# spectrseq/spectrseqtools

Hardware: AMD Instinct MI355X
Metric: peaks explained/sec (full 148-nt alphabet, <=20-mer) at 1/2/4/8 MI355X (higher is better)
Workload: dtype u64; 1 GPU; config3: synthetic spectra (SURVEY 8(d)), full 104-mass/105-row alphabet, <=20-mer, A7 (4 breakages/peak) + A8 (sliding-window differences) per step; spectra_per_gpu=10000, max_len=20, max_modifications=10, a7_stream=engine stream, parallelism=1 GPU

## Files before the change

include/sst.h:

```cpp
#ifndef SST_H
#define SST_H

#include <stdint.h>

#ifdef __cplusplus
extern "C" {
#endif

#define SST_OK 0
#define SST_E_ARG (-1)
#define SST_E_HIP (-2)
#define SST_E_NOMEM (-3)
#define SST_E_TABLE (-4)
#define SST_E_INTERNAL (-5)

#define SST_NONE 0
#define SST_EMPTY 1
#define SST_SOME 2
#define SST_OUT_OF_TABLE (-1)
#define SST_OVERFLOW (-2)
#define SST_ABORTED (-4)


typedef struct sst_ctx sst_ctx;
// ... 68 lines not shown
int sst_step_rows_device(sst_table* t, const double* d_obs, const int64_t* d_peak_off, int64_t n_spec,
                         int64_t n_peaks, const double* d_intensity, double intensity_cutoff, double mass_cutoff,
                         const double* d_su_seq, const double* shifts, const uint8_t* sides, int n_shifts,
                         double max_weight, double tolerance, double precision, int64_t max_mods_scalar,
                         uint64_t cap_per_query, int64_t max_queries, int8_t* d_valid_out, sst_result** out);
int sst_result_queries(sst_result* r, int64_t* n);

int sst_result_settle(sst_result* r, uint64_t* n_hits, uint64_t* payload_bytes);

int sst_result_host(sst_result* r, const int8_t** status, const uint64_t** count, const uint64_t** offset,
                    const uint8_t** payload, uint64_t* payload_bytes);
int sst_result_device(sst_result* r, int8_t** d_status, uint64_t** d_count, uint64_t** d_offset,
                      uint8_t** d_payload, uint64_t* payload_bytes);
int sst_result_hit_list(sst_result* r, void** d_hits, uint64_t* n_hits);
int sst_result_pair_hits(sst_result* r, void** d_refs, uint64_t* n_pair_hits, uint64_t* pair_bytes, int* n_scan_wg);
int sst_table_pair_records(sst_table* t, uint32_t* recs, int64_t cap, int64_t* n);
int64_t sst_wire_pack(sst_result* r, const int8_t* d_valid, int64_t n_valid, void* d_out, int64_t cap);
int sst_result_fetch(sst_result* r);
void sst_result_free(sst_result* r);

int sst_result_stats(const sst_result* r, uint64_t* stats_out );

#define SST_LB_EMPTY_WINDOW (-5)
int sst_length_bound_alpha_batch(sst_table* t, const double* su_mass, const double* obs_mass, const int32_t* spec,
                                 const uint64_t* alpha, int64_t n_alpha, int64_t n, double tolerance,
                                 double precision, int max_len, int64_t max_mods, int direction, int64_t* out,
                                 int8_t* status);
#define SST_LB_EXACT_ONLY 2
#define SST_LB_REPLAY 4
int sst_length_bound_batch(sst_table* t, const double* su_mass, const double* obs_mass, int64_t n, double tolerance,
// ... 314 lines not shown
```

spectrseqtools_amd/_native.py:

```python
import ctypes
import os
import threading

import numpy as np

_HERE = os.path.dirname(os.path.abspath(__file__))
LIB_PATH = os.environ.get("SST_LIBRARY", os.path.join(_HERE, "libsstgpu.so"))

SST_NONE, SST_EMPTY, SST_SOME = 0, 1, 2
SST_OUT_OF_TABLE, SST_OVERFLOW, SST_ABORTED = -1, -2, -4
SST_LB_EMPTY_WINDOW = -5

EXPORTS = (
    "sst_device_count", "sst_ctx_create", "sst_ctx_destroy", "sst_last_error", "sst_ctx_stream",
    "sst_ctx_synchronize", "sst_table_build", "sst_table_upload", "sst_table_set_budgets", "sst_table_shape",
    "sst_table_download", "sst_table_destroy", "sst_is_valid_batch", "sst_is_valid_batch_device",
    "sst_explain_batch", "sst_explain_batch_device", "sst_explain_alpha_batch_device", "sst_explain_alpha_lens_batch_device", "sst_result_host", "sst_result_device", "sst_result_fetch",
    "sst_result_free", "sst_result_stats", "sst_profile_enable", "sst_profile_select",
    "sst_profile_sample", "sst_profile_read", "sst_length_bound_batch", "sst_explain_recursion_batch", "sst_is_singleton_batch",
    "sst_is_singleton_batch_device", "sst_ctx_set_stream", "sst_result_hit_list", "sst_result_settle",
    "sst_window_pairs", "sst_is_valid_peaks", "sst_is_valid_peaks_device", "sst_result_pair_hits",
    "sst_table_pair_records", "sst_su_diff_queries", "sst_sort_rows", "sst_step_device",
    "sst_wire_pack", "sst_explain_pairs_alpha", "sst_explain_pairs_alpha_device", "sst_is_valid_alpha",
    "sst_is_valid_alpha_device", "sst_dict_union", "sst_step_rows_device", "sst_result_queries",
    "sst_classify_rows_device", "sst_fix_round_device", "sst_valid_rows_alpha_device",
    "sst_bins_count_device", "sst_bins_emit_device", "sst_length_bound_alpha_batch",
    "sst_py_tuple_hash", "sst_pyset_order", "sst_pyset_table_size", "sst_walk_scratch_bytes",
    "sst_skel_walk_device", "sst_result_refs_device", "sst_dict_count_device", "sst_dict_build_device",
    "sst_reach_rows_device", "sst_length_bounds_reach_device", "sst_jaccard_device", "sst_skeleton_alpha_device",
    "sst_dict_list_device", "sst_fix_finish_device", "sst_pipe_reserve_rows", "sst_reach_lowest_device",
    "sst_length_bounds_frontier_device", "sst_post_skeleton_device", "sst_ctx_trim", "sst_requery_merge_device",
    "sst_handoff_count_device", "sst_handoff_emit_device",
)

K_IS_VALID, K_EXPLAIN_SCAN, K_EXPLAIN_DEEP, K_EXPLAIN_NOMEMO, K_EXPLAIN_EXACT, K_EXPLAIN_EXPAND = 0, 1, 2, 3, 4, 5
K_RESULT_PACK = 6
(K_CLASSIFY_ROWS, K_FIX_ROUND, K_VALID_ALPHA, K_BINS_COUNT, K_BINS_EMIT, K_DICT, K_SKEL_WALK, K_REACH_ROWS,
 K_LENGTH_BOUND, K_JACCARD, K_PAIRS_ALPHA, K_REQUERY_MERGE, K_HANDOFF) = range(7, 20)
K_COUNT = 24
KERNEL_NAMES = {K_IS_VALID: "k_is_valid", K_EXPLAIN_SCAN: "k_explain_scan", K_EXPLAIN_DEEP: "k_explain_deferred",
                K_EXPLAIN_EXPAND: "k_explain_expand",
                K_RESULT_PACK: "k_result_pack",
                K_CLASSIFY_ROWS: "k_classify_rows", K_FIX_ROUND: "k_fix_round", K_VALID_ALPHA: "k_valid_alpha",
                K_BINS_COUNT: "k_bins_count", K_BINS_EMIT: "k_bins_emit", K_DICT: "k_dict_build",
                K_SKEL_WALK: "k_skel_walk", K_REACH_ROWS: "k_reach_rows", K_LENGTH_BOUND: "k_length_bound",
                K_JACCARD: "k_jaccard", K_PAIRS_ALPHA: "k_pairs_alpha", K_REQUERY_MERGE: "k_requery_merge",
                K_HANDOFF: "k_handoff"}
# ... 156 lines not shown
    lib.sst_profile_enable.argtypes = [_P, _I]
    lib.sst_profile_select.argtypes = [_P, ctypes.c_uint32]
    lib.sst_profile_sample.argtypes = [_P, ctypes.c_uint32]
    lib.sst_profile_read.argtypes = [_P, _P, _P]
    lib.sst_length_bound_batch.argtypes = [_P, _P, _P, _I64, _D, _D, _I, _I64, _I, _P, _P]
    lib.sst_length_bound_alpha_batch.argtypes = [_P, _P, _P, _P, _P, _I64, _I64, _D, _D, _I, _I64, _I, _P, _P]
    lib.sst_explain_recursion_batch.argtypes = [_P, _P, _P, _I64, _D, _D, _P, _I64, _U64, _PP]
    lib.sst_is_singleton_batch.argtypes = [_P, _P, _I, _P, _P, _I64, _D, _D, _P]
    lib.sst_is_singleton_batch_device.argtypes = [_P, _P, _I, _P, _P, _I64, _D, _D, _P]
    lib.sst_is_valid_peaks.argtypes = [_P, _P, _I64, _P, _I, _D, _D, _P]
    lib.sst_is_valid_peaks_device.argtypes = [_P, _P, _I64, _P, _I, _D, _D, _P]
    lib.sst_window_pairs.argtypes = [_P, _P, _I64, _D, _P, _P, _I64]
    lib.sst_window_pairs.restype = _I64
    lib.sst_result_pair_hits.argtypes = [_P, _PP, ctypes.POINTER(_U64), ctypes.POINTER(_U64), ctypes.POINTER(_I)]
    lib.sst_result_pair_hits.restype = _I
    lib.sst_table_pair_records.argtypes = [_P, _P, _I64, ctypes.POINTER(_I64)]
    lib.sst_table_pair_records.restype = _I
    lib.sst_wire_pack.argtypes = [_P, _P, _I64, _P, _I64]
    lib.sst_wire_pack.restype = _I64
    lib.sst_su_diff_queries.argtypes = [_P, _P, _P, _P, _I64, _D, _D, _P, _P, _P, _P, _I64]
    lib.sst_su_diff_queries.restype = _I64
    lib.sst_py_tuple_hash.argtypes = [_P, _I64]
    lib.sst_py_tuple_hash.restype = _I64
    lib.sst_pyset_order.argtypes = [_P, _P, _I64, _P]
    lib.sst_pyset_order.restype = _I64
    lib.sst_sort_rows.argtypes = [_P, _P, _I64, _I64, _P]
    lib.sst_sort_rows.restype = _I
    lib.sst_step_device.argtypes = [_P, _P, _I64, _P, _I, _P, _P, _P, _I64, _D, _D, _P, _I64, _I, _U64, _PP]
    lib.sst_step_device.restype = _I
    lib.sst_explain_pairs_alpha.argtypes = [_P, _P, _P, _P, _P, _I64, _I64, _D, _D, _P, _P, _P, _P]
# ... 400 lines not shown
    def _wrap(cls, engine, h, w):
        nr, nc, C = _I(), _I64(), _I()
        engine._lib.sst_table_shape(h, ctypes.byref(nr), ctypes.byref(nc), ctypes.byref(C))
        return cls(engine, h, nr.value, nc.value, C.value, w.tolist())

    def set_budgets(self, is_mod, caps):
        key = (tuple(bool(x) for x in is_mod), tuple(int(c) for c in caps))
        if key == self._budgets:
            return
        m = np.ascontiguousarray(key[0], dtype=np.uint8)
        c = np.ascontiguousarray(key[1], dtype=np.int64)
        self.engine.check(self.engine._lib.sst_table_set_budgets(self.handle, _ptr(m), _ptr(c)),
                          "sst_table_set_budgets")
        self._budgets = key

    def pair_records(self):
        L = self.engine._lib
        n = _I64()
        self.engine.check(L.sst_table_pair_records(self.handle, None, 0, ctypes.byref(n)), "sst_table_pair_records")
        out = np.zeros(n.value, np.uint32)
        if n.value:
            self.engine.check(L.sst_table_pair_records(self.handle, _ptr(out), n.value, ctypes.byref(n)),
                              "sst_table_pair_records")
        return out

    def download(self):
        out = np.empty((self.n_rows, self.n_cols), dtype=_DT[self.compression])
        self.engine.check(self.engine._lib.sst_table_download(self.handle, _ptr(out)), "sst_table_download")
        return out

# ... 241 lines not shown
```

spectrseqtools_amd/csrc/sst_api.cpp:

```cpp
#include <hip/hip_runtime.h>
#include <sched.h>

#include <algorithm>
#include <atomic>
#include <chrono>
#include <cmath>
#include <cstdio>
#include <cstdlib>
#include <cstring>
#include <mutex>
#include <string>
#include <thread>
#include <vector>

#include "sst.h"
#include "sst_internal.h"
#include "sst_pyset.h"

using namespace sst;

namespace {

struct DevBuf {
  void* p = nullptr;
// ... 47 lines not shown
  DevBuf ws_deep;
  DevBuf ws_hash, ws_frames, ws_stacks, ws_epochs;
  DevBuf singleton_masses;
  struct LbfWs {
    DevBuf flags, lpar, lval, gtab, ctab, glist, ctl, bstart, bgroups, qi, qrow, roots, ncnt, grec, crec, ngrp;
    uint64_t S = 0, ncap = 0, budget = 0;
    bool by_default = false;
    int epoch = 0;
    bool dirty = true;
    uint64_t done_q = 0, done_nodes = 0;
    double band_frac = 0.3;
  } lbf, lbf_small;
  uint32_t hash_cap = 0;
  int exact_blocks = 0;
  int n_cu = 256;
  int expand_blocks = 0;
  uint32_t prof = 0;
  struct Pending {
    int kid;
    hipEvent_t a, b;
  };
  std::vector<Pending> pending;
  std::vector<hipEvent_t> pool;
  double prof_ms[SST_K_COUNT] = {0};
  int64_t prof_n[SST_K_COUNT] = {0};
  uint32_t prof_every = 1;
  uint64_t prof_seen[SST_K_COUNT] = {0};
  DevBuf pipe_big;
  uint32_t pipe_big_rows = 0, pipe_big_slots = 0;
  int pipe_big_wg = 0;
// ... 2 lines not shown
struct sst_table {
  sst_ctx* ctx = nullptr;
  int n_rows = 0;
  int64_t n_cols = 0;
  int C = 32;
  int64_t M = 0;
  std::vector<int64_t> masses;
  std::vector<uint8_t> is_mod;
  std::vector<int64_t> cap;
  DevBuf packed, index, valid, w, capd, modd, pairs, census, canon_c;
  int64_t canon_c_words = 0;
  std::vector<uint32_t> pair_recs;
  uint64_t pair_key = 0;
  bool pair_key_set = false;
  int scan_blocks = 0;
  bool closure = false;
  TableArgs args{};
};

struct LenBudgets {
  const int32_t* qlen = nullptr;
  const int32_t* caps = nullptr;
  const uint64_t* capz = nullptr;
  const uint32_t* never = nullptr;
};

struct sst_result {
  sst_ctx* ctx = nullptr;
  int64_t n = 0;
  int64_t cap_n = 0;
// ... 313 lines not shown
  *out = nullptr;
  int n = sst_device_count();
  if (device < 0 || device >= n) return SST_E_ARG;
  sst_ctx* c = new sst_ctx();
  c->device = device;
  {
    int cu = 0;
    if (hipDeviceGetAttribute(&cu, hipDeviceAttributeMultiprocessorCount, device) == hipSuccess && cu > 0) c->n_cu = cu;
    (void)hipGetLastError();
  }
  if (hipSetDevice(device) != hipSuccess || hipStreamCreateWithFlags(&c->own, hipStreamNonBlocking) != hipSuccess) {
    delete c;
    return SST_E_HIP;
  }
  c->stream = c->own;
  *out = c;
  return SST_OK;
}

void sst_ctx_destroy(sst_ctx* c) {
  if (!c) return;
  (void)hipSetDevice(c->device);
  (void)hipStreamSynchronize(c->stream);
  (void)hipStreamSynchronize(c->own);
  for (DevBuf* b : {&c->in_mass, &c->in_thr, &c->in_mods, &c->out_valid, &c->ws_deep, &c->ws_hash, &c->ws_frames,
                    &c->ws_stacks, &c->ws_epochs, &c->singleton_masses})
    b->release();
  prof_resolve(c);
  for (hipEvent_t e : c->pool) (void)hipEventDestroy(e);
  (void)hipStreamDestroy(c->own);
// ... 532 lines not shown
  fold_scan_limits(ta, q);
  q.alpha = d_alpha;
  q.spec = d_spec;
  q.comp = (int)t->C;
  q.qlen = lb.qlen;
  q.caps_len = lb.caps;
  q.capz_len = lb.capz;
  q.never_len = lb.never;
  OutArgs o = out_args(r);
  const bool fused = !eager_tail && !r->bitset_scan;
  r->fused_pass = fused;
  r->scan_hdr_pending = fused;
  r->scan_hits = r->scan_bytes = 0;
  if (fused) {
    o.fused = 1;
    o.pass_id = ++r->pack_seq;
#ifdef SST_DIAG
    static const char* dbg = getenv("SST_PACK_DBG");
    o.dbg = dbg ? atoi(dbg) : 0;
#endif
  }
  const bool step = peaks && peaks->n > 0 && peaks->n_shifts == 4 && fused;
  if (peaks && peaks->n > 0 && peaks->n_shifts > 0 && !step) {
    Prof p(c, SST_K_IS_VALID);
    HIP_OK(c, launch_is_valid_peaks(t->args.valid, t->args.limit, t->args.full_lo, t->args.full_hi,
                                    t->args.first_reach, peaks->obs, peaks->n, peaks->shifts, peaks->n_shifts, tol,
                                    prec, peaks->out, c->stream));
  }
  {
    Prof p(c, SST_K_EXPLAIN_MAIN);
// ... 10 lines not shown
    eager_tail = true;
  }
  if (eager_tail)
    if (int rc = launch_tail(t, r)) return rc;
  return launch_pack(r);
}

int step_scan_wg_per_cu() {
  static const int v = [] {
    const char* e = getenv("SST_STEP_SCAN_WG_PER_CU");
    return e && atoi(e) > 0 ? atoi(e) : 1;
  }();
  return v;
}

int alloc_result(sst_table* t, int64_t n, sst_result** out, bool step = false) {
  sst_ctx* c = t->ctx;
  if (t->scan_blocks == 0) t->scan_blocks = c->n_cu * explain_scan_blocks_per_cu(scan_dyn_lds(t->args));
  if (c->expand_blocks == 0) c->expand_blocks = c->n_cu * explain_expand_blocks_per_cu();
  sst_result* r = new sst_result();
  r->ctx = c;
  r->pass_stream = c->stream;
  r->n = n;
  r->cap_n = n;
  size_t nn = (size_t)std::max<int64_t>(n, 1);
  int64_t tiles = ((int64_t)nn + 63) / 64;
  const int64_t grid = step ? (int64_t)c->n_cu * std::min<int64_t>(t->scan_blocks / c->n_cu, step_scan_wg_per_cu())
                            : (int64_t)t->scan_blocks;
  r->n_wg = (int)std::max<int64_t>(1, std::min<int64_t>(grid, (tiles + 15) / 16));
  r->n_scan_waves = (int64_t)r->n_wg * (kScanWG / 64);
  r->work_region = (uint64_t)((tiles + r->n_scan_waves - 1) / r->n_scan_waves) * 64;
  r->n_expand_waves = c->expand_blocks * (kWG / 64);
  r->region_bytes = std::max<uint64_t>(2048, round16(16 * r->work_region));
// ... 611 lines not shown
  *n_hits = r->n_hits;
  return SST_OK;
}

int sst_result_pair_hits(sst_result* r, void** d_refs, uint64_t* n_pair_hits, uint64_t* pair_bytes, int* n_scan_wg) {
  if (!r) return SST_E_ARG;
  sst_ctx* c = r->ctx;
  std::lock_guard<std::recursive_mutex> g(c->mu);
  if (int rc = set_device(c)) return rc;
  if (int rc = settle(r)) return rc;
  if (int rc = order_after_settle(r)) return rc;
  if (d_refs) *d_refs = r->refs.p;
  if (n_pair_hits) *n_pair_hits = r->scan_hits;
  if (pair_bytes) *pair_bytes = r->scan_bytes;
  if (n_scan_wg) *n_scan_wg = r->rows_pass ? 0 : r->n_wg;
  return SST_OK;
}

int sst_table_pair_records(sst_table* t, uint32_t* recs, int64_t cap, int64_t* n) {
  if (!t || !n) return SST_E_ARG;
  *n = t->args.pairs_enabled ? (int64_t)t->pair_recs.size() : 0;
  if (!recs || *n == 0) return SST_OK;
  if (cap < *n) return fail(t->ctx, SST_E_ARG, "pair records: buffer too small");
  memcpy(recs, t->pair_recs.data(), (size_t)*n * 4);
  return SST_OK;
}

static uint64_t pair_key_of(const std::vector<uint32_t>& recs) {
  uint64_t h = 0xCBF29CE484222325ull;
  const uint8_t* p = (const uint8_t*)recs.data();
// ... 1727 lines not shown
```

spectrseqtools_amd/csrc/sst_internal.h:

```cpp
#pragma once
#include <hip/hip_runtime.h>
#include <stddef.h>
#include <stdint.h>

#include <type_traits>

#include "sst.h"

namespace sst {

constexpr int kMaxRows = 120;
static_assert(kMaxRows == SST_MAX_ROWS, "the ABI's row stride");
constexpr int kWG = 256;
#ifndef SST_DEF_WG
#define SST_DEF_WG 256
#endif
constexpr int kDefWG = SST_DEF_WG;
constexpr int kShallowDepth = 4;
constexpr int kMaxDepth = 96;
constexpr int kInfBudget = 1 << 30;
constexpr int kScanWG = 1024;
constexpr int kMaxSingletonMasses = 1024;
constexpr int kMaxPairLds = 44 * 1024;
constexpr uint32_t kItemZero = 1u, kItemUnclassified = 2u, kItemNever = 4u;
// ... 90 lines not shown
  uint32_t* counters;
  uint32_t* lists;
  unsigned long long* stats;
  uint4* dhits;
  uint32_t* dhit_count;
  int fused;
  uint64_t* agg;
  uint64_t* agg_next;
  uint4* hits_out;
  uint16_t* hit_refs;
  uint8_t* dense;
  uint64_t* hdr;
  uint64_t* hdr_host;
  uint64_t pass_id;
  int dbg;
};

constexpr uint32_t kHitOffsetFlag = 1u << 31;

enum {
  kCtlCursor = 0,
  kCtlCounters = 1,
  kCtlExactRetries = 3,
  kCtlArenaRetries = 13,
  kCtlRegionNeed = 14,
  kCtlStats = 256,
  kCtlDhits = 512,
  kCtlWords = 1024
};

enum {
// ... 425 lines not shown
                           const double* mass, const double* thr, int64_t n, double tol, double prec, int8_t* out,
                           hipStream_t st);
hipError_t launch_is_valid_peaks(const uint64_t* valid, int64_t limit, int64_t full_lo, int64_t full_hi,
                                 int64_t first_reach, const double* obs, int64_t n, const double* shifts, int n_w,
                                 double tol, double prec, int8_t* out, hipStream_t st);
hipError_t launch_step(const TableArgs& t, const QueryArgs& q, const OutArgs& o, int n_blocks, const double* obs,
                       int64_t n_peaks, const double* shifts4, double tol, double prec, int8_t* valid_out,
                       hipStream_t st);
hipError_t launch_explain_scan(const TableArgs& t, const QueryArgs& q, const OutArgs& o, int n_blocks,
                               hipStream_t st);
hipError_t launch_explain_expand(const TableArgs& t, const QueryArgs& q, const OutArgs& o, int n_blocks,
                                 hipStream_t st);
int explain_scan_blocks_per_cu(size_t dyn_lds);
int explain_expand_blocks_per_cu();
size_t scan_dyn_lds(const TableArgs& t);
hipError_t launch_result_pack(const PackArgs& p, hipStream_t st);
hipError_t launch_hits_to_arrays(const uint4* hits, uint64_t n_hits, const int8_t* status, uint64_t* count,
                                 uint64_t* offset, hipStream_t st);
hipError_t launch_explain_deferred(const TableArgs& t, const QueryArgs& q, const OutArgs& o, void* ws_deep,
                                   int shallow_blocks, int deep_blocks, const ExactWs& ws, int exact_blocks,
                                   hipStream_t st);
size_t glob_frame_bytes();
hipError_t launch_layer_step(const uint64_t* prev, uint64_t* next, int64_t nwords, const int* w, int n_rows,
                             hipStream_t st);
hipError_t launch_length_bound(const TableArgs& t, const LBArgs& q, char* hash, int8_t* vals, char* frames,
                               uint32_t hash_cap, int exact_units, bool fast_pass, hipStream_t st);
size_t lb_frame_bytes();
hipError_t launch_is_singleton(const int64_t* masses, int n_masses, const double* mass, const double* thr, int64_t n,
                               double tol, double prec, int8_t* out, hipStream_t st);
hipError_t launch_explain_recursion(const TableArgs& t, const QueryArgs& q, const OutArgs& o, char* hash,
// ... 8 lines not shown
```

spectrseqtools_amd/csrc/sst_kernels.hip:

```cpp
#include <hip/hip_runtime.h>
#include <stdint.h>

#include <algorithm>

#include "sst_internal.h"
#include "sst_quant.h"

namespace sst {

struct M128 {
  uint64_t a, b;
};
__device__ __forceinline__ M128 rows_upto(int r) {
  M128 m;
  if (r >= 63) {
    m.a = ~0ull;
    int k = r - 63;
    m.b = k >= 64 ? ~0ull : ((1ull << k) - 1ull);
  } else {
    m.a = r < 0 ? 0ull : ((2ull << r) - 1ull);
    m.b = 0;
  }
  return m;
}
// ... 1463 lines not shown
  asm volatile("" : "+s"(p));
  return p;
}
template <typename T>
__device__ __forceinline__ T karg_load(KargPtr p, size_t off) {
  static_assert(std::is_trivially_copyable<T>::value, "kernarg members are plain data");
  T v;
  __builtin_memcpy(&v, (const __attribute__((address_space(4))) T*)(p + off), sizeof(T));
  return v;
}
#define SCAN_KARG(p, member) \
  karg_load<std::remove_cv_t<decltype(((ScanArgs*)nullptr)->member)>>(p, offsetof(ScanArgs, member))

template <bool THR, bool MODS>
__device__ __forceinline__ void scan_end_phase(uint32_t bid, uint32_t nbid, uint32_t w_in, int lane, uint32_t n_hit,
                                               uint32_t n_staged, uint32_t n_work, uint32_t st_q,
                                               uint32_t st_payload);

template <bool THR, bool MODS>
__device__ __forceinline__ void explain_scan_wg(const ScanArgs& a, const uint32_t bid, const uint32_t nbid) {
  const TableArgs& t = a.t;
  const QueryArgs& q = a.q;
  const OutArgs& out = a.out;
  extern __shared__ uint32_t lds_pair_img[];
  if (bid == 0) {
    if (threadIdx.x < (unsigned)out.ctl_words) out.ctl_next[threadIdx.x] = 0;
    for (uint32_t k = threadIdx.x; k < nbid; k += blockDim.x) out.agg_next[k] = 0;
  }
  const int n_img = 2 * (t.n_pairs + 2) + t.n_buckets;
  static_assert(kMaxPairLds <= kImgPieces * kScanWG * 16, "the image is staged in kImgPieces pieces per lane");
  const uint32_t n_img16 = (uint32_t)(n_img + 3) >> 2;
  const __amdgpu_buffer_rsrc_t img_rsrc = buf_rsrc(t.pair_data, n_img16 * 16u);
  u32x4 img[kImgPieces];
#pragma unroll
  for (int j = 0; j < kImgPieces; ++j)
    img[j] = __builtin_amdgcn_raw_buffer_load_b128(img_rsrc, (threadIdx.x + j * kScanWG) * 16u, 0, 0);
  const PairLds pl = scan_pair_lds(lds_pair_img, t.n_pairs, t.pair_base, t.pair_shift);
  const int lane = threadIdx.x & 63;
  const uint32_t w_in = __builtin_amdgcn_readfirstlane(threadIdx.x >> 6);
  const uint32_t wave = bid * (kScanWG / 64) + w_in;
  const uint32_t n_waves = nbid * (kScanWG / 64);
  const uint32_t n = (uint32_t)q.n;
  const uint32_t ntiles = (n + 63) >> 6;
  const double limitf = (double)t.limit;
  uint32_t st_q = 0, st_payload = 0;
  uint4* wl = out.work + (uint64_t)wave * out.work_region;
  uint32_t n_work = 0;
  const uint32_t wl_bytes = (uint32_t)(out.work_region * 16);
  const __amdgpu_buffer_rsrc_t wl_rsrc = buf_rsrc(wl, wl_bytes);
  const __amdgpu_buffer_rsrc_t st_rsrc = buf_rsrc(out.status, n);
  uint32_t n_hit = 0;
  uint32_t n_staged = 0;
  auto fetch = [&](uint32_t tl, double& m, double& tt, int64_t& mm) {
    const uint32_t j = tl < ntiles ? min(tl * 64 + lane, n - 1) : n - 1;
    m = __builtin_nontemporal_load(q_at(q.mass, j));
    if (THR) tt = __builtin_nontemporal_load(q_at(q.thr, j));
    if (MODS) mm = __builtin_nontemporal_load(q_at(q.max_mods, j));
  };
  auto step = [&](uint32_t tile, double m_in, double t_in, int64_t mm_cur) {
    const uint32_t i = tile * 64 + lane;
    const bool live = i < n;
    const double m_cur = m_in, t_cur = THR ? t_in : q.tol * m_in;
    double lof, hif;
    quantise_lean_fn(m_cur, t_cur, [] { return SCAN_KARG(scan_karg(), q.prec); }, q.rprec, lof, hif);
    const bool nonempty = live && lof <= hif;
    const bool oot = nonempty && !(hif < limitf);
    const bool zero = nonempty && !oot && lof <= 0.0 && hif >= 0.0;
    const double af = __builtin_fmax(lof, 1.0);
    const bool active = nonempty && !oot && af <= hif;
    const uint32_t a = active ? (uint32_t)af : 0u, hi = active ? (uint32_t)hif : 0u;
    bool pair, a0ok = true;
    if (MODS) {
      const int A0 = clamp_budget(mm_cur);
      a0ok = !t.any_mod || A0 >= kInfBudget || (uint64_t)hi < (uint64_t)(A0 + 1) * (uint64_t)t.w_min_mod;
      pair = active && a0ok && hi < t.pair_lim;
    } else {
      pair = active && hi < q.pair_hi_lim;
    }
    const bool work = active && !pair;
    uint32_t first = 0, cnt = 0, bytes = 0;
    if (pair) cnt = pair_walk(pl, a, hi, first, bytes);
    int8_t status = oot ? (int8_t)SST_OUT_OF_TABLE : (zero ? (int8_t)SST_EMPTY : (int8_t)SST_NONE);
    if (cnt) status = cnt > q.cap32 ? (int8_t)SST_OVERFLOW : (int8_t)SST_SOME;
    st_payload += status == SST_SOME ? bytes + 2u : 0u;
    st_q += pair ? 1u : 0u;
    const uint64_t hbal = __ballot(cnt != 0);
    const uint32_t hpos = n_hit + mbcnt(hbal);
    __builtin_amdgcn_raw_buffer_store_b8((uint8_t)status, st_rsrc, (live && !work) ? i : kBufSkip, 0, 0);
    const u32x2 rv = {i, first | (cnt << 16)};
    __builtin_amdgcn_raw_buffer_store_b64(rv, wl_rsrc, cnt ? wl_bytes - 8u * (hpos + 1u) : kBufSkip, 0, 0);
    n_hit += (uint32_t)__builtin_popcountll(hbal);
    if (__ballot(work)) {
      const KargPtr ka = scan_karg();
      bool never;
      if (MODS) {
        const int32_t* const qlen = SCAN_KARG(ka, q.qlen);
        const uint32_t nl = qlen ? SCAN_KARG(ka, q.never_len)[qlen[live ? i : n - 1]] : SCAN_KARG(ka, t.never_lim);
        never = a0ok && hi < nl;
      } else {
        never = hi < SCAN_KARG(ka, q.never_hi_lim);
      }
      int cls = -1;
      if (work) {
        if (never && hi < SCAN_KARG(ka, t.shallow_hi)) {
          cls = kClassShallow;
        } else {
          cls = never ? kClassDeep : (SCAN_KARG(ka, q.with_memo) ? kClassExact : kClassNomemo);
          SCAN_KARG(ka, out.status)[i] = (int8_t)kStatusPending;
        }
      }
      uint32_t* const stage = SCAN_KARG(ka, out.stage) + (uint64_t)wave * SCAN_KARG(ka, out.work_region);
      const uint64_t cb = __ballot(cls >= 0);
      if (cls >= 0) stage[n_staged + mbcnt(cb)] = i | ((uint32_t)cls << 30);
      n_staged += (uint32_t)__builtin_popcountll(cb);
    }
  };
  double mA = 0.0, tA = 0.0, mB = 0.0, tB = 0.0;
  int64_t mmA = q.max_mods_scalar, mmB = q.max_mods_scalar;
  const uint32_t vw = (((w_in >> 1) * nbid + bid) << 1) | (w_in & 1u);
  fetch(vw, mA, tA, mmA);
  __builtin_amdgcn_raw_buffer_store_b8(0, st_rsrc, kBufSkip, 0, 0);
  __builtin_amdgcn_raw_buffer_store_b8(1, st_rsrc, kBufSkip + 64u, 0, 0);
  fetch(vw + n_waves, mB, tB, mmB);
#pragma unroll
  for (int j = 0; j < kImgPieces; ++j)
    if (threadIdx.x + j * kScanWG < n_img16) ((u32x4*)lds_pair_img)[threadIdx.x + j * kScanWG] = img[j];
  __syncthreads();
  for (uint32_t tile = vw; tile < ntiles; tile += 2 * n_waves) {
    step(tile, mA, tA, mmA);
    fetch(tile + 2 * n_waves, mA, tA, mmA);
    if (tile + n_waves >= ntiles) break;
    step(tile + n_waves, mB, tB, mmB);
    fetch(tile + 3 * n_waves, mB, tB, mmB);
  }
  scan_end_phase<THR, MODS>(bid, nbid, w_in, lane, n_hit, n_staged, n_work, st_q, st_payload);
}

template <bool THR, bool MODS>
__device__ __forceinline__ void scan_end_phase(const uint32_t bid, const uint32_t nbid, const uint32_t w_in,
                                               const int lane, const uint32_t n_hit, const uint32_t n_staged,
                                               const uint32_t n_work, const uint32_t st_q,
                                               const uint32_t st_payload) {
  extern __shared__ uint32_t lds_pair_img[];
  const KargPtr ka = scan_karg();
  const OutArgs out = SCAN_KARG(ka, out);
  struct {
    int64_t n;
    uint32_t cap32;
  } const q{SCAN_KARG(ka, q.n), SCAN_KARG(ka, q.cap32)};
  const PairLds pl = scan_pair_lds(lds_pair_img, SCAN_KARG(ka, t.n_pairs), SCAN_KARG(ka, t.pair_base),
                                   SCAN_KARG(ka, t.pair_shift));
  const uint32_t wave = bid * (kScanWG / 64) + w_in;
  uint4* const wl = out.work + (uint64_t)wave * out.work_region;
  uint32_t* const stage = out.stage + (uint64_t)wave * out.work_region;
  const uint32_t pay = wave_sum32(st_payload);
  const uint64_t region0 = (uint64_t)wave * out.region_bytes;
  const bool fits = out.fused || pay <= min(out.region_bytes, (uint64_t)UINT32_MAX);
  const uint32_t units = fits ? (pay + 15u) >> 4 : 0u;
  if (lane == 0) {
    out.work_count[wave] = n_work;
    out.tally[wave] = make_uint2(n_hit, units);
    if (!fits) {
      atomicAdd(out.arena_retries, (unsigned long long)max(n_hit, 1u));
      atomicMax(out.region_need, (unsigned long long)pay);
    }
  }
  wave_stats_flush(out, wave, lane, kStatPair, kStatPairPayload, st_q, st_payload);
  __shared__ uint2 wg_part[kScanWG / 64];
  __shared__ uint32_t wg_pre[2];
  __shared__ uint32_t wg_cls[kScanWG / 64][kNumClasses];
  __shared__ uint32_t wg_cls_base[kNumClasses];
  asm volatile("s_waitcnt vmcnt(0)" ::: "memory");
  uint32_t n_cls[kNumClasses] = {0u, 0u, 0u, 0u};
  for (uint32_t k0 = 0; k0 < n_staged; k0 += 64) {
    const uint32_t k = k0 + lane;
    const uint32_t cl = k < n_staged ? stage[k] >> 30 : 4u;
#pragma unroll
    for (int c = 0; c < kNumClasses; ++c) n_cls[c] += (uint32_t)__builtin_popcountll(__ballot(cl == (uint32_t)c));
  }
  if (lane == 0) {
    wg_part[w_in] = make_uint2(n_hit, units);
#pragma unroll
    for (int c = 0; c < kNumClasses; ++c) wg_cls[w_in][c] = n_cls[c];
  }
  __syncthreads();
  uint32_t wg_h = 0, wg_u = 0;
// ... 2 lines not shown
    for (int k = 0; k < kScanWG / 64; ++k) tot += wg_cls[k][threadIdx.x];
    wg_cls_base[threadIdx.x] = tot ? atomicAdd(&out.counters[threadIdx.x], tot) : 0u;
  }
  if (threadIdx.x == 0) {
    asm volatile("s_waitcnt vmcnt(0)" ::: "memory");
    for (int k = 0; k < kScanWG / 64; ++k) {
      wg_h += wg_part[k].x;
      wg_u += wg_part[k].y;
    }
    out.wg_tally[bid] = make_uint2(wg_h, wg_u);
    if (out.fused)
      __hip_atomic_store(out.agg + bid, (1ull << 63) | ((uint64_t)wg_u << 32) | wg_h, __ATOMIC_RELAXED,
                         __HIP_MEMORY_SCOPE_AGENT);
  }
  const uint2* rec = (const uint2*)(wl + out.work_region);
  const uint32_t nh_copy = (out.dbg & 1) ? 0 : n_hit;
  uint2 rr[kPreChunks];
  uint32_t pbv[kPreChunks], inclv[kPreChunks], rel[kPreChunks + 1];
  rel[0] = 0;
#pragma unroll
  for (int c = 0; c < kPreChunks; ++c) {
    const uint32_t k = c * 64 + lane;
    rr[c] = k < nh_copy ? *(rec - 1 - k) : make_uint2(0, 0);
  }
#pragma unroll
  for (int c = 0; c < kPreChunks; ++c) {
    const uint32_t k = c * 64 + lane, cnt = rr[c].y >> 16;
    pbv[c] = (k < nh_copy && cnt <= q.cap32) ? pair_bytes(pl, rr[c].y & 0xFFFFu, cnt) + 2u : 0u;
    inclv[c] = wave_incl_scan32(pbv[c]);
    rel[c + 1] = rel[c] + (uint32_t)__builtin_amdgcn_readlane((int)inclv[c], 63);
  }
  uint64_t hbase = 0, pbase = region0;
  if (out.fused) {
    if (w_in == 0) {
      const uint32_t b = bid;
      uint32_t ph = 0, pu = 0;
      for (uint32_t k0 = 0; k0 < b; k0 += 64) {
        const uint32_t k = k0 + lane;
// ... 72 lines not shown
      if (out.fused) {
        const uint64_t word = pb ? off : (uint64_t)cnt;
        out.hits_out[hbase + k] = make_uint4(r.x, cnt, (uint32_t)word, (uint32_t)(word >> 32));
        out.hit_refs[hbase + k] = (uint16_t)(first | (pb ? 0u : 0x8000u));
      } else {
        *((uint2*)rec - 1 - k) = make_uint2(r.x, cnt | (pb << 16));
      }
    }
  };
#pragma unroll
  for (int c = 0; c < kPreChunks; ++c)
    if (c * 64 < nh_copy) emit(c * 64 + lane, rr[c], pbv[c], pbase + rel[c] + (inclv[c] - pbv[c]));
  uint64_t run = pbase + rel[kPreChunks];
  for (uint32_t k0 = kPreChunks * 64; k0 < nh_copy; k0 += 64) {
    const uint32_t k = k0 + lane;
    const uint2 r = k < n_hit ? *(rec - 1 - k) : make_uint2(0, 0);
    const uint32_t cnt = r.y >> 16;
    const uint32_t pb = (k < n_hit && cnt <= q.cap32) ? pair_bytes(pl, r.y & 0xFFFFu, cnt) + 2u : 0u;
    const uint32_t incl = wave_incl_scan32(pb);
    emit(k, r, pb, run + (incl - pb));
    run += (uint32_t)__builtin_amdgcn_readlane((int)incl, 63);
  }
}
template <bool THR, bool MODS>
__global__ __launch_bounds__(kScanWG, 8) void k_explain_scan(ScanArgs a) {
  explain_scan_wg<THR, MODS>(a, blockIdx.x, gridDim.x);
}
template <bool THR, bool MODS>
__global__ __launch_bounds__(kScanWG, 8) void k_step(StepArgs a) {
  const uint32_t n_scan = gridDim.x - a.a7_blocks;
  if (blockIdx.x >= n_scan) {
// ... 1513 lines not shown
        if (m == 4) hipLaunchKernelGGL(k_is_valid_peaks<4>, dim3(grid), dim3(256), 0, st, v2, s2);
        if (m == 3) hipLaunchKernelGGL(k_is_valid_peaks<3>, dim3(grid), dim3(256), 0, st, v2, s2);
        if (m == 2) hipLaunchKernelGGL(k_is_valid_peaks<2>, dim3(grid), dim3(256), 0, st, v2, s2);
        if (m == 1) hipLaunchKernelGGL(k_is_valid_peaks<1>, dim3(grid), dim3(256), 0, st, v2, s2);
      }
  }
  return hipGetLastError();
}
size_t scan_dyn_lds(const TableArgs& t) {
  if (!t.pairs_enabled) return 0;
  return ((size_t)(2 * (t.n_pairs + 2) + t.n_buckets) * sizeof(uint32_t) + 15) / 16 * 16;
}
hipError_t launch_explain_scan(const TableArgs& t, const QueryArgs& q, const OutArgs& o, int n_blocks,
                               hipStream_t st) {
  if (q.n <= 0) return hipSuccess;
  const size_t dyn = scan_dyn_lds(t);
  const ScanArgs a{t, q, o};
  if (!t.pairs_enabled)
    hipLaunchKernelGGL(k_bitset_scan, dim3(n_blocks), dim3(kScanWG), 0, st, t, q, o);
  else if (q.thr && q.max_mods)
    hipLaunchKernelGGL((k_explain_scan<true, true>), dim3(n_blocks), dim3(kScanWG), dyn, st, a);
  else if (q.thr)
    hipLaunchKernelGGL((k_explain_scan<true, false>), dim3(n_blocks), dim3(kScanWG), dyn, st, a);
  else if (q.max_mods)
    hipLaunchKernelGGL((k_explain_scan<false, true>), dim3(n_blocks), dim3(kScanWG), dyn, st, a);
  else
    hipLaunchKernelGGL((k_explain_scan<false, false>), dim3(n_blocks), dim3(kScanWG), dyn, st, a);
  return hipGetLastError();
}
hipError_t launch_step(const TableArgs& t, const QueryArgs& q, const OutArgs& o, int n_blocks, const double* obs,
                       int64_t n_peaks, const double* shifts4, double tol, double prec, int8_t* valid_out,
                       hipStream_t st) {
  if (!t.pairs_enabled || q.n <= 0) return hipErrorInvalidValue;
  const size_t dyn = scan_dyn_lds(t);
  ValidArgs v{t.valid, t.limit, t.full_lo, t.full_hi, t.first_reach, obs, nullptr, n_peaks, tol, prec, 1.0 / prec,
              valid_out};
  PeakShifts sh{};
  for (int k = 0; k < 4; ++k) sh.shift[k] = shifts4[k];
  const uint32_t a7 = (uint32_t)((n_peaks + kScanWG - 1) / kScanWG);
  const dim3 grid(a7 + (uint32_t)n_blocks);
  const StepArgs a{{t, q, o}, v, sh, a7};
  if (q.thr && q.max_mods)
    hipLaunchKernelGGL((k_step<true, true>), grid, dim3(kScanWG), dyn, st, a);
  else if (q.thr)
    hipLaunchKernelGGL((k_step<true, false>), grid, dim3(kScanWG), dyn, st, a);
  else if (q.max_mods)
    hipLaunchKernelGGL((k_step<false, true>), grid, dim3(kScanWG), dyn, st, a);
  else
    hipLaunchKernelGGL((k_step<false, false>), grid, dim3(kScanWG), dyn, st, a);
// ... 5 lines not shown
  hipLaunchKernelGGL(k_explain_expand, dim3(n_blocks), dim3(kWG), 0, st, t, q, o);
  return hipGetLastError();
}
static int occupancy(const void* k, int threads, size_t dyn) {
  int nb = 0;
  if (hipOccupancyMaxActiveBlocksPerMultiprocessor(&nb, k, threads, dyn) != hipSuccess) {
    (void)hipGetLastError();
    return 1;
  }
  return nb > 0 ? nb : 1;
}
int explain_scan_blocks_per_cu(size_t dyn) {
  return dyn ? occupancy((const void*)k_explain_scan<true, false>, kScanWG, dyn)
             : occupancy((const void*)k_bitset_scan, kScanWG, 0);
}
int explain_expand_blocks_per_cu() { return occupancy((const void*)k_explain_expand, kWG, 0); }
hipError_t launch_result_pack(const PackArgs& p, hipStream_t st) {
  hipLaunchKernelGGL(k_result_pack, dim3(p.n_wg > 0 ? p.n_wg : 1), dim3(1024), 0, st, p);
  return hipGetLastError();
}
hipError_t launch_hits_to_arrays(const uint4* hits, uint64_t n_hits, const int8_t* status, uint64_t* count,
                                 uint64_t* offset, hipStream_t st) {
  if (n_hits == 0) return hipSuccess;
  hipLaunchKernelGGL(k_hits_to_arrays, dim3(blocks_for((int64_t)n_hits, 256)), dim3(256), 0, st, hits, n_hits, status,
                     count, offset);
  return hipGetLastError();
}
hipError_t launch_wire_pack(const WireArgs& a, hipStream_t st) {
  if (a.be_e == 0) return hipSuccess;
  hipLaunchKernelGGL(k_wire_pack, dim3(a.be_e), dim3(256), 0, st, a);
// ... 62 lines not shown
```

Before: 17.19 billion peaks/s.

## Stage scan hit records in spare LDS instead of global worklist

The explain scan now packs each wave's hit records (pair-list index, lane, tile ordinal, count) into a per-wave LDS slot carved from unused dynamic LDS, falling back to the global worklist once the slot fills or a field overflows. The end phase reads hits back from LDS first, then from global memory. The goal is to remove the global 8-byte store and reload per hit. The host raises the kernels' dynamic LDS limit to half of a CU's LDS and sizes the slot so occupancy is not reduced. It also simplifies the tile loop bounds and the class-staging logic, at the cost of extra LDS use and more complex record encoding.

```diff
diff --git a/include/sst.h b/include/sst.h
--- a/include/sst.h
+++ b/include/sst.h
@@ -106,6 +106,7 @@
                       uint8_t** d_payload, uint64_t* payload_bytes);
 int sst_result_hit_list(sst_result* r, void** d_hits, uint64_t* n_hits);
 int sst_result_pair_hits(sst_result* r, void** d_refs, uint64_t* n_pair_hits, uint64_t* pair_bytes, int* n_scan_wg);
+int sst_table_scan_lds_hits(sst_table* t, uint32_t* per_wave);
 int sst_table_pair_records(sst_table* t, uint32_t* recs, int64_t cap, int64_t* n);
 int64_t sst_wire_pack(sst_result* r, const int8_t* d_valid, int64_t n_valid, void* d_out, int64_t cap);
 int sst_result_fetch(sst_result* r);
diff --git a/spectrseqtools_amd/_native.py b/spectrseqtools_amd/_native.py
--- a/spectrseqtools_amd/_native.py
+++ b/spectrseqtools_amd/_native.py
@@ -30,7 +30,7 @@
     "sst_reach_rows_device", "sst_length_bounds_reach_device", "sst_jaccard_device", "sst_skeleton_alpha_device",
     "sst_dict_list_device", "sst_fix_finish_device", "sst_pipe_reserve_rows", "sst_reach_lowest_device",
     "sst_length_bounds_frontier_device", "sst_post_skeleton_device", "sst_ctx_trim", "sst_requery_merge_device",
-    "sst_handoff_count_device", "sst_handoff_emit_device",
+    "sst_handoff_count_device", "sst_handoff_emit_device", "sst_table_scan_lds_hits",
 )
 
 K_IS_VALID, K_EXPLAIN_SCAN, K_EXPLAIN_DEEP, K_EXPLAIN_NOMEMO, K_EXPLAIN_EXACT, K_EXPLAIN_EXPAND = 0, 1, 2, 3, 4, 5
@@ -217,6 +217,8 @@
     lib.sst_window_pairs.restype = _I64
     lib.sst_result_pair_hits.argtypes = [_P, _PP, ctypes.POINTER(_U64), ctypes.POINTER(_U64), ctypes.POINTER(_I)]
     lib.sst_result_pair_hits.restype = _I
+    lib.sst_table_scan_lds_hits.argtypes = [_P, ctypes.POINTER(ctypes.c_uint32)]
+    lib.sst_table_scan_lds_hits.restype = _I
     lib.sst_table_pair_records.argtypes = [_P, _P, _I64, ctypes.POINTER(_I64)]
     lib.sst_table_pair_records.restype = _I
     lib.sst_wire_pack.argtypes = [_P, _P, _I64, _P, _I64]
@@ -647,6 +649,12 @@
                           "sst_table_set_budgets")
         self._budgets = key
 
+    def scan_lds_hits(self):
+        k = ctypes.c_uint32()
+        self.engine.check(self.engine._lib.sst_table_scan_lds_hits(self.handle, ctypes.byref(k)),
+                          "sst_table_scan_lds_hits")
+        return int(k.value)
+
     def pair_records(self):
         L = self.engine._lib
         n = _I64()
diff --git a/spectrseqtools_amd/csrc/sst_api.cpp b/spectrseqtools_amd/csrc/sst_api.cpp
--- a/spectrseqtools_amd/csrc/sst_api.cpp
+++ b/spectrseqtools_amd/csrc/sst_api.cpp
@@ -85,6 +85,7 @@
   uint32_t hash_cap = 0;
   int exact_blocks = 0;
   int n_cu = 256;
+  size_t scan_dyn_max = 64 * 1024;
   int expand_blocks = 0;
   uint32_t prof = 0;
   struct Pending {
@@ -117,6 +118,7 @@
   uint64_t pair_key = 0;
   bool pair_key_set = false;
   int scan_blocks = 0;
+  uint32_t lds_hits = 0;
   bool closure = false;
   TableArgs args{};
 };
@@ -460,6 +462,7 @@
     return SST_E_HIP;
   }
   c->stream = c->own;
+  c->scan_dyn_max = sst::scan_allow_large_lds();
   *out = c;
   return SST_OK;
 }
@@ -1022,6 +1025,7 @@
   r->scan_hits = r->scan_bytes = 0;
   if (fused) {
     o.fused = 1;
+    o.lds_hits = t->lds_hits;
     o.pass_id = ++r->pack_seq;
 #ifdef SST_DIAG
     static const char* dbg = getenv("SST_PACK_DBG");
@@ -1062,9 +1066,24 @@
   return v;
 }
 
+uint32_t scan_lds_hits(size_t img_lds, size_t dyn_max) {
+  static const long forced = [] {
+    const char* e = getenv("SST_SCAN_LDS_HITS");
+    return e && *e ? atol(e) : -1L;
+  }();
+  const uint32_t most = scan_lds_hits_max(img_lds, dyn_max);
+  return forced >= 0 ? (uint32_t)std::min<long>(forced, (long)most) : most;
+}
+
+void size_scan(sst_table* t) {
+  if (t->scan_blocks) return;
+  t->scan_blocks = t->ctx->n_cu * explain_scan_blocks_per_cu(scan_dyn_lds(t->args));
+  t->lds_hits = scan_lds_hits(scan_dyn_lds(t->args), t->ctx->scan_dyn_max);
+}
+
 int alloc_result(sst_table* t, int64_t n, sst_result** out, bool step = false) {
   sst_ctx* c = t->ctx;
-  if (t->scan_blocks == 0) t->scan_blocks = c->n_cu * explain_scan_blocks_per_cu(scan_dyn_lds(t->args));
+  size_scan(t);
   if (c->expand_blocks == 0) c->expand_blocks = c->n_cu * explain_expand_blocks_per_cu();
   sst_result* r = new sst_result();
   r->ctx = c;
@@ -1706,6 +1725,16 @@
   if (n_pair_hits) *n_pair_hits = r->scan_hits;
   if (pair_bytes) *pair_bytes = r->scan_bytes;
   if (n_scan_wg) *n_scan_wg = r->rows_pass ? 0 : r->n_wg;
+  return SST_OK;
+}
+
+int sst_table_scan_lds_hits(sst_table* t, uint32_t* per_wave) {
+  if (!t || !per_wave) return SST_E_ARG;
+  sst_ctx* c = t->ctx;
+  std::lock_guard<std::recursive_mutex> g(c->mu);
+  if (int rc = set_device(c)) return rc;
+  size_scan(t);
+  *per_wave = t->lds_hits;
   return SST_OK;
 }
 
diff --git a/spectrseqtools_amd/csrc/sst_internal.h b/spectrseqtools_amd/csrc/sst_internal.h
--- a/spectrseqtools_amd/csrc/sst_internal.h
+++ b/spectrseqtools_amd/csrc/sst_internal.h
@@ -128,7 +128,21 @@
   uint64_t* hdr_host;
   uint64_t pass_id;
   int dbg;
-};
+  uint32_t lds_hits;
+};
+
+constexpr int kHitFirstBits = 13, kHitLaneBits = 6, kHitOrdBits = 13;
+constexpr uint32_t kHitMaxCount = 255, kHitMaxOrd = (1u << kHitOrdBits) - 1u;
+static_assert(kMaxPairLds / 8 <= (1 << kHitFirstBits), "a pair-list entry index fits the LDS hit record");
+static_assert(kHitFirstBits + kHitLaneBits + kHitOrdBits == 32, "the LDS hit record's fields");
+constexpr size_t kCuLdsBytes = 160 * 1024;
+constexpr uint32_t scan_hit_slot_bytes(uint32_t lds_hits) { return 4u * lds_hits + ((lds_hits + 3u) & ~3u); }
+inline size_t scan_hit_lds_bytes(uint32_t lds_hits) {
+  return (size_t)scan_hit_slot_bytes(lds_hits) * (kScanWG / 64);
+}
+__host__ __device__ inline uint32_t scan_hit_slot(uint32_t lds_hits, uint32_t w_in) {
+  return w_in * scan_hit_slot_bytes(lds_hits) + ((lds_hits + 3u) & ~3u);
+}
 
 constexpr uint32_t kHitOffsetFlag = 1u << 31;
 
@@ -584,6 +598,8 @@
 int explain_scan_blocks_per_cu(size_t dyn_lds);
 int explain_expand_blocks_per_cu();
 size_t scan_dyn_lds(const TableArgs& t);
+size_t scan_allow_large_lds();
+uint32_t scan_lds_hits_max(size_t img_lds, size_t dyn_max);
 hipError_t launch_result_pack(const PackArgs& p, hipStream_t st);
 hipError_t launch_hits_to_arrays(const uint4* hits, uint64_t n_hits, const int8_t* status, uint64_t* count,
                                  uint64_t* offset, hipStream_t st);
diff --git a/spectrseqtools_amd/csrc/sst_kernels.hip b/spectrseqtools_amd/csrc/sst_kernels.hip
--- a/spectrseqtools_amd/csrc/sst_kernels.hip
+++ b/spectrseqtools_amd/csrc/sst_kernels.hip
@@ -1501,7 +1501,7 @@
 
 template <bool THR, bool MODS>
 __device__ __forceinline__ void scan_end_phase(uint32_t bid, uint32_t nbid, uint32_t w_in, int lane, uint32_t n_hit,
-                                               uint32_t n_staged, uint32_t n_work, uint32_t st_q,
+                                               uint32_t lds_end, uint32_t n_staged, uint32_t n_work, uint32_t st_q,
                                                uint32_t st_payload);
 
 template <bool THR, bool MODS>
@@ -1528,7 +1528,8 @@
   const uint32_t wave = bid * (kScanWG / 64) + w_in;
   const uint32_t n_waves = nbid * (kScanWG / 64);
   const uint32_t n = (uint32_t)q.n;
-  const uint32_t ntiles = (n + 63) >> 6;
+  const uint32_t n1 = n - 1;
+  auto has_tile = [&](uint32_t tl) { return (tl << 6) <= n1; };
   const double limitf = (double)t.limit;
   uint32_t st_q = 0, st_payload = 0;
   uint4* wl = out.work + (uint64_t)wave * out.work_region;
@@ -1537,16 +1538,20 @@
   const __amdgpu_buffer_rsrc_t wl_rsrc = buf_rsrc(wl, wl_bytes);
   const __amdgpu_buffer_rsrc_t st_rsrc = buf_rsrc(out.status, n);
   uint32_t n_hit = 0;
+  uint8_t* const hit_slot = (uint8_t*)lds_pair_img + n_img16 * 16u + scan_hit_slot(out.lds_hits, w_in);
+  uint32_t lds_end = out.lds_hits;
+  uint32_t ord = 0;
+  const uint32_t w_min_mod = t.any_mod ? (uint32_t)t.w_min_mod : UINT32_MAX;
   uint32_t n_staged = 0;
   auto fetch = [&](uint32_t tl, double& m, double& tt, int64_t& mm) {
-    const uint32_t j = tl < ntiles ? min(tl * 64 + lane, n - 1) : n - 1;
+    const uint32_t j = min(tl * 64 + lane, n1);
     m = __builtin_nontemporal_load(q_at(q.mass, j));
     if (THR) tt = __builtin_nontemporal_load(q_at(q.thr, j));
     if (MODS) mm = __builtin_nontemporal_load(q_at(q.max_mods, j));
   };
   auto step = [&](uint32_t tile, double m_in, double t_in, int64_t mm_cur) {
     const uint32_t i = tile * 64 + lane;
-    const bool live = i < n;
+    const bool live = i <= n1;
     const double m_cur = m_in, t_cur = THR ? t_in : q.tol * m_in;
     double lof, hif;
     quantise_lean_fn(m_cur, t_cur, [] { return SCAN_KARG(scan_karg(), q.prec); }, q.rprec, lof, hif);
@@ -1559,7 +1564,7 @@
     bool pair, a0ok = true;
     if (MODS) {
       const int A0 = clamp_budget(mm_cur);
-      a0ok = !t.any_mod || A0 >= kInfBudget || (uint64_t)hi < (uint64_t)(A0 + 1) * (uint64_t)t.w_min_mod;
+      a0ok = A0 >= kInfBudget || (uint64_t)hi < (uint64_t)(A0 + 1) * (uint64_t)w_min_mod;
       pair = active && a0ok && hi < t.pair_lim;
     } else {
       pair = active && hi < q.pair_hi_lim;
@@ -1573,32 +1578,37 @@
     st_q += pair ? 1u : 0u;
     const uint64_t hbal = __ballot(cnt != 0);
     const uint32_t hpos = n_hit + mbcnt(hbal);
+    const uint32_t n_hit1 = n_hit + (uint32_t)__builtin_popcountll(hbal);
+    const bool keep = n_hit1 <= lds_end && !__ballot(cnt > kHitMaxCount) && ord <= kHitMaxOrd;
+    if (!keep) lds_end = min(lds_end, n_hit);
     __builtin_amdgcn_raw_buffer_store_b8((uint8_t)status, st_rsrc, (live && !work) ? i : kBufSkip, 0, 0);
-    const u32x2 rv = {i, first | (cnt << 16)};
-    __builtin_amdgcn_raw_buffer_store_b64(rv, wl_rsrc, cnt ? wl_bytes - 8u * (hpos + 1u) : kBufSkip, 0, 0);
-    n_hit += (uint32_t)__builtin_popcountll(hbal);
+    if (cnt && keep) {
+      ((uint32_t*)hit_slot)[hpos] = first | ((uint32_t)lane << kHitFirstBits) | (ord << (kHitFirstBits + kHitLaneBits));
+      *(hit_slot - 1 - hpos) = (uint8_t)cnt;
+    }
+    if (!keep && hbal) {
+      const u32x2 rv = {i, first | (cnt << 16)};
+      __builtin_amdgcn_raw_buffer_store_b64(rv, wl_rsrc, cnt ? wl_bytes - 8u * (hpos + 1u) : kBufSkip, 0, 0);
+    }
+    n_hit = n_hit1;
+    ++ord;
     if (__ballot(work)) {
       const KargPtr ka = scan_karg();
       bool never;
       if (MODS) {
         const int32_t* const qlen = SCAN_KARG(ka, q.qlen);
-        const uint32_t nl = qlen ? SCAN_KARG(ka, q.never_len)[qlen[live ? i : n - 1]] : SCAN_KARG(ka, t.never_lim);
+        const uint32_t nl = qlen ? SCAN_KARG(ka, q.never_len)[qlen[live ? i : n1]] : SCAN_KARG(ka, t.never_lim);
         never = a0ok && hi < nl;
       } else {
         never = hi < SCAN_KARG(ka, q.never_hi_lim);
       }
-      int cls = -1;
-      if (work) {
-        if (never && hi < SCAN_KARG(ka, t.shallow_hi)) {
-          cls = kClassShallow;
-        } else {
-          cls = never ? kClassDeep : (SCAN_KARG(ka, q.with_memo) ? kClassExact : kClassNomemo);
-          SCAN_KARG(ka, out.status)[i] = (int8_t)kStatusPending;
-        }
-      }
+      const bool shallow = never && hi < SCAN_KARG(ka, t.shallow_hi);
+      const uint32_t deferred = never ? kClassDeep : (SCAN_KARG(ka, q.with_memo) ? kClassExact : kClassNomemo);
+      const uint32_t cls = shallow ? (uint32_t)kClassShallow : deferred;
+      if (work && !shallow) SCAN_KARG(ka, out.status)[i] = (int8_t)kStatusPending;
       uint32_t* const stage = SCAN_KARG(ka, out.stage) + (uint64_t)wave * SCAN_KARG(ka, out.work_region);
-      const uint64_t cb = __ballot(cls >= 0);
-      if (cls >= 0) stage[n_staged + mbcnt(cb)] = i | ((uint32_t)cls << 30);
+      const uint64_t cb = __ballot(work);
+      if (work) stage[n_staged + mbcnt(cb)] = i | (cls << 30);
       n_staged += (uint32_t)__builtin_popcountll(cb);
     }
   };
@@ -1613,20 +1623,22 @@
   for (int j = 0; j < kImgPieces; ++j)
     if (threadIdx.x + j * kScanWG < n_img16) ((u32x4*)lds_pair_img)[threadIdx.x + j * kScanWG] = img[j];
   __syncthreads();
-  for (uint32_t tile = vw; tile < ntiles; tile += 2 * n_waves) {
+  for (uint32_t tile = vw; has_tile(tile);) {
+    const uint32_t t1 = tile + n_waves, t2 = t1 + n_waves;
     step(tile, mA, tA, mmA);
-    fetch(tile + 2 * n_waves, mA, tA, mmA);
-    if (tile + n_waves >= ntiles) break;
-    step(tile + n_waves, mB, tB, mmB);
-    fetch(tile + 3 * n_waves, mB, tB, mmB);
-  }
-  scan_end_phase<THR, MODS>(bid, nbid, w_in, lane, n_hit, n_staged, n_work, st_q, st_payload);
+    fetch(t2, mA, tA, mmA);
+    if (!has_tile(t1)) break;
+    step(t1, mB, tB, mmB);
+    fetch(t2 + n_waves, mB, tB, mmB);
+    tile = t2;
+  }
+  scan_end_phase<THR, MODS>(bid, nbid, w_in, lane, n_hit, lds_end, n_staged, n_work, st_q, st_payload);
 }
 
 template <bool THR, bool MODS>
 __device__ __forceinline__ void scan_end_phase(const uint32_t bid, const uint32_t nbid, const uint32_t w_in,
-                                               const int lane, const uint32_t n_hit, const uint32_t n_staged,
-                                               const uint32_t n_work, const uint32_t st_q,
+                                               const int lane, const uint32_t n_hit, const uint32_t lds_end,
+                                               const uint32_t n_staged, const uint32_t n_work, const uint32_t st_q,
                                                const uint32_t st_payload) {
   extern __shared__ uint32_t lds_pair_img[];
   const KargPtr ka = scan_karg();
@@ -1657,6 +1669,7 @@
   __shared__ uint32_t wg_pre[2];
   __shared__ uint32_t wg_cls[kScanWG / 64][kNumClasses];
   __shared__ uint32_t wg_cls_base[kNumClasses];
+  const uint32_t k_lds = min(lds_end, n_hit);
   asm volatile("s_waitcnt vmcnt(0)" ::: "memory");
   uint32_t n_cls[kNumClasses] = {0u, 0u, 0u, 0u};
   for (uint32_t k0 = 0; k0 < n_staged; k0 += 64) {
@@ -1689,6 +1702,17 @@
                          __HIP_MEMORY_SCOPE_AGENT);
   }
   const uint2* rec = (const uint2*)(wl + out.work_region);
+  const uint32_t n_img16 = (uint32_t)(2 * (SCAN_KARG(ka, t.n_pairs) + 2) + SCAN_KARG(ka, t.n_buckets) + 3) >> 2;
+  const uint8_t* const hit_slot = (const uint8_t*)lds_pair_img + n_img16 * 16u + scan_hit_slot(out.lds_hits, w_in);
+  const uint32_t vw = (((w_in >> 1) * nbid + bid) << 1) | (w_in & 1u), n_waves = nbid * (kScanWG / 64);
+  auto hit_rec = [&](uint32_t k) {
+    if (k < k_lds) {
+      const uint32_t w = ((const uint32_t*)hit_slot)[k], c = *(hit_slot - 1 - k);
+      const uint32_t tile = vw + (w >> (kHitFirstBits + kHitLaneBits)) * n_waves;
+      return make_uint2(tile * 64u + ((w >> kHitFirstBits) & 63u), (w & ((1u << kHitFirstBits) - 1u)) | (c << 16));
+    }
+    return *(rec - 1 - k);
+  };
   const uint32_t nh_copy = (out.dbg & 1) ? 0 : n_hit;
   uint2 rr[kPreChunks];
   uint32_t pbv[kPreChunks], inclv[kPreChunks], rel[kPreChunks + 1];
@@ -1696,7 +1720,7 @@
 #pragma unroll
   for (int c = 0; c < kPreChunks; ++c) {
     const uint32_t k = c * 64 + lane;
-    rr[c] = k < nh_copy ? *(rec - 1 - k) : make_uint2(0, 0);
+    rr[c] = k < nh_copy ? hit_rec(k) : make_uint2(0, 0);
   }
 #pragma unroll
   for (int c = 0; c < kPreChunks; ++c) {
@@ -1799,7 +1823,7 @@
   uint64_t run = pbase + rel[kPreChunks];
   for (uint32_t k0 = kPreChunks * 64; k0 < nh_copy; k0 += 64) {
     const uint32_t k = k0 + lane;
-    const uint2 r = k < n_hit ? *(rec - 1 - k) : make_uint2(0, 0);
+    const uint2 r = k < n_hit ? hit_rec(k) : make_uint2(0, 0);
     const uint32_t cnt = r.y >> 16;
     const uint32_t pb = (k < n_hit && cnt <= q.cap32) ? pair_bytes(pl, r.y & 0xFFFFu, cnt) + 2u : 0u;
     const uint32_t incl = wave_incl_scan32(pb);
@@ -3343,7 +3367,7 @@
 hipError_t launch_explain_scan(const TableArgs& t, const QueryArgs& q, const OutArgs& o, int n_blocks,
                                hipStream_t st) {
   if (q.n <= 0) return hipSuccess;
-  const size_t dyn = scan_dyn_lds(t);
+  const size_t dyn = scan_dyn_lds(t) + scan_hit_lds_bytes(o.lds_hits);
   const ScanArgs a{t, q, o};
   if (!t.pairs_enabled)
     hipLaunchKernelGGL(k_bitset_scan, dim3(n_blocks), dim3(kScanWG), 0, st, t, q, o);
@@ -3361,7 +3385,7 @@
                        int64_t n_peaks, const double* shifts4, double tol, double prec, int8_t* valid_out,
                        hipStream_t st) {
   if (!t.pairs_enabled || q.n <= 0) return hipErrorInvalidValue;
-  const size_t dyn = scan_dyn_lds(t);
+  const size_t dyn = scan_dyn_lds(t) + scan_hit_lds_bytes(o.lds_hits);
   ValidArgs v{t.valid, t.limit, t.full_lo, t.full_hi, t.first_reach, obs, nullptr, n_peaks, tol, prec, 1.0 / prec,
               valid_out};
   PeakShifts sh{};
@@ -3397,6 +3421,38 @@
   return dyn ? occupancy((const void*)k_explain_scan<true, false>, kScanWG, dyn)
              : occupancy((const void*)k_bitset_scan, kScanWG, 0);
 }
+static const void* const kScanKernels[] = {
+    (const void*)k_explain_scan<false, false>, (const void*)k_explain_scan<false, true>,
+    (const void*)k_explain_scan<true, false>,  (const void*)k_explain_scan<true, true>,
+    (const void*)k_step<false, false>,         (const void*)k_step<false, true>,
+    (const void*)k_step<true, false>,          (const void*)k_step<true, true>};
+size_t scan_allow_large_lds() {
+  bool ok = true;
+  for (const void* k : kScanKernels)
+    ok = hipFuncSetAttribute(k, hipFuncAttributeMaxDynamicSharedMemorySize, (int)(kCuLdsBytes / 2)) == hipSuccess && ok;
+  (void)hipGetLastError();
+  return ok ? kCuLdsBytes / 2 : 64 * 1024;
+}
+uint32_t scan_lds_hits_max(size_t img, size_t dyn_max) {
+  if (!img) return 0;
+  size_t stat = 0;
+  for (const void* k : kScanKernels) {
+    hipFuncAttributes fa{};
+    if (hipFuncGetAttributes(&fa, k) == hipSuccess) stat = std::max(stat, (size_t)fa.sharedSizeBytes);
+  }
+  (void)hipGetLastError();
+  const size_t room = std::min(kCuLdsBytes / 2, dyn_max + stat);
+  if (img + stat + 16 > room) return 0;
+  uint32_t K = (uint32_t)((room - img - stat - 16) / scan_hit_lds_bytes(4)) * 4u;
+  const int want = explain_scan_blocks_per_cu(img);
+  auto fits = [&](uint32_t k) {
+    const size_t dyn = img + scan_hit_lds_bytes(k);
+    return explain_scan_blocks_per_cu(dyn) >= want &&
+           occupancy((const void*)k_step<true, false>, kScanWG, dyn) >= std::min(want, 2);
+  };
+  while (K > 0 && !fits(K)) K = K > 16 ? K - 16 : 0;
+  return K;
+}
 int explain_expand_blocks_per_cu() { return occupancy((const void*)k_explain_expand, kWG, 0); }
 hipError_t launch_result_pack(const PackArgs& p, hipStream_t st) {
   hipLaunchKernelGGL(k_result_pack, dim3(p.n_wg > 0 ? p.n_wg : 1), dim3(1024), 0, st, p);
```

Result: faster. 17.71 billion peaks/s, median of 6 (+3.0%).
